# plindhorst/Ray-Tracing-Project

Measured on AMD Instinct MI355X. Metric: Mrays/s (primary) + frame ms at 1920x1080, 1M-tri BVH, 1/2/4/8 GPU, higher is better.
Workload: dtype f32; 1 GPU; C3: 1000000 random triangles (SplitMix64 seed 12345), 1920x1080 primary rays, eye (0,0,1), 1 light; frame=1920x1080, triangles=1000000, mode=primary, parallelism=tiles/1 (one GPU, whole frame), launcher=none, frames_in_flight=4, prewarm_frames=200, hw_queues=4, bvh_nodes=1145398, bvh_depth=26, ref_boxes=4480, builder=sbvh-gpu

## Files before the change

ray-tracing-project_amd/csrc/rt_builders.cpp:

```cpp
#include <atomic>
#include <chrono>
#include <cstdio>
#include <cstdlib>
#include <cstring>
#include <future>

#include "rt_host.h"

namespace rt {
namespace {
struct Prim {
  float lo[3], hi[3], c[3];
  uint32_t id;
};

static bool take_task(std::atomic<int>& live, unsigned cap) {
  if (live.fetch_add(1) < (int)cap) return true;
  live.fetch_sub(1);
  return false;
}

constexpr int kBins = 32;
constexpr float kIsect = 1.0f;
struct Bins {
// ... 88 lines not shown
        const float s = sc[axis];
        const float lo = cb.lo[axis];
        auto it = std::partition(prims.begin() + b, prims.begin() + e, [&](const Prim& p) {
          return std::min(kBins - 1, (int)((p.c[axis] - lo) * s)) <= best_bin;
        });
        mid = (uint32_t)(it - prims.begin());
      }
    } else if ((int)n <= leaf_size) {
      return make_leaf_h();
    }
    if (axis < 0 || mid == b || mid == e) {
      if ((int)n <= kMaxLeaf && !(ext[0] > 0 || ext[1] > 0 || ext[2] > 0)) return make_leaf_h();
      int k = (ext[0] >= ext[1] && ext[0] >= ext[2]) ? 0 : (ext[1] >= ext[2] ? 1 : 2);
      mid = b + n / 2;
      std::nth_element(prims.begin() + b, prims.begin() + mid, prims.begin() + e,
                       [&](const Prim& x, const Prim& y) { return x.c[k] < y.c[k]; });
    }
    const uint32_t me = next.fetch_add(1);
    Aabb lb, rb;
    uint32_t lh, rh;
    if (n > 4096 && depth < 16 && take_task(tasks, hw)) {
      auto fut = std::async(std::launch::async, [&]() { return build(b, mid, depth + 1, lb); });
      rh = build(mid, e, depth + 1, rb);
      lh = fut.get();
      tasks.fetch_sub(1);
    } else {
      lh = build(b, mid, depth + 1, lb);
      rh = build(mid, e, depth + 1, rb);
    }
    Node64 nd{};
    set_child(nd, 0, lb, pad, lh);
    set_child(nd, 1, rb, pad, rh);
    nodes[me] = nd;
    return me;
  }
};

struct SbvhBuilder {
  const HostScene& hs;
  std::vector<Node64>& nodes;
  std::vector<std::vector<uint32_t>> leaf_lists;
  std::atomic<uint32_t> next{0}, nleaf{0};
  std::atomic<int64_t> refs{0};
  int leaf_size = 4;
  float pad = 0.0f, kTrav = 0.7f, alpha = 1e-5f, root_area = 1.0f;
  std::atomic<int> max_depth{0};
  std::atomic<int> tasks{0};
  unsigned hw = 1;

  void verts(uint32_t f, double v[3][3]) const {
    for (int j = 0; j < 3; j++) {
      const f3& w = bound_vert(hs, f, j);
      v[j][0] = w.x; v[j][1] = w.y; v[j][2] = w.z;
    }
  }
  static float down(double x) { float f = (float)x; return (double)f > x ? std::nextafter(f, -INFINITY) : f; }
  static float up(double x) { float f = (float)x; return (double)f < x ? std::nextafter(f, INFINITY) : f; }
  bool clip(uint32_t f, int k, float a, float b, const Prim& within, Prim& out) const {
    double v[3][3];
    verts(f, v);
    double lo[3] = {INFINITY, INFINITY, INFINITY}, hi[3] = {-INFINITY, -INFINITY, -INFINITY};
    auto add = [&](const double* q) {
      for (int i = 0; i < 3; i++) { lo[i] = std::min(lo[i], q[i]); hi[i] = std::max(hi[i], q[i]); }
    };
    for (int j = 0; j < 3; j++) {
      const double* p = v[j];
      const double* q = v[(j + 1) % 3];
      if (p[k] >= a && p[k] <= b) add(p);
      for (double pl : {(double)a, (double)b}) {
        if ((p[k] < pl && q[k] > pl) || (p[k] > pl && q[k] < pl)) {
          const double t = (pl - p[k]) / (q[k] - p[k]);
          double x[3];
          for (int i = 0; i < 3; i++) x[i] = p[i] + t * (q[i] - p[i]);
          x[k] = pl;
          add(x);
        }
      }
    }
    out.id = f;
    for (int i = 0; i < 3; i++) {
      out.lo[i] = std::max(down(lo[i]), within.lo[i]);
      out.hi[i] = std::min(up(hi[i]), within.hi[i]);
      if (i == k) { out.lo[i] = std::max(out.lo[i], a); out.hi[i] = std::min(out.hi[i], b); }
      if (!(out.lo[i] <= out.hi[i])) return false;
      out.c[i] = 0.5f * (out.lo[i] + out.hi[i]);
    }
    return true;
  }

  uint32_t leaf(std::vector<Prim>& r) {
    const uint32_t li = nleaf.fetch_add(1);
    std::vector<uint32_t>& ids = leaf_lists[li];
    ids.reserve(r.size());
    for (const Prim& p : r) ids.push_back(p.id);
    const uint32_t n = (uint32_t)r.size();
    std::vector<Prim>().swap(r);
    return make_leaf(li, n);
  }

  uint32_t build(std::vector<Prim>& r, int depth, Aabb& box, int64_t budget) {
    const uint32_t n = (uint32_t)r.size();
    Aabb cb;
    box = Aabb();
    {
      Aabb pb[16], pc[16];
      const int T = parallel_chunks(n, [&](size_t b, size_t e, int t) {
        Aabb a, c;
        for (size_t i = b; i < e; i++) { a.grow(r[i].lo, r[i].hi); c.growp(r[i].c); }
        pb[t] = a;
        pc[t] = c;
      });
      for (int t = 0; t < T; t++) { box.merge(pb[t]); cb.merge(pc[t]); }
    }
    int md = max_depth.load();
    while (depth > md && !max_depth.compare_exchange_weak(md, depth)) {}
    if (n == 1) return leaf(r);
    const bool forced = depth >= kMaxDepth - 20;
    const float parent_area = std::max(box.area(), 1e-30f);
    const int TB = chunk_count(n);
    std::vector<Bins> part((size_t)TB);
    int o_axis = -1, o_bin = -1;
    float o_cost = INFINITY;
    Aabb o_lb, o_rb;
    float ext[3], sc[3];
    for (int k = 0; k < 3; k++) { ext[k] = cb.hi[k] - cb.lo[k]; sc[k] = ext[k] > 0.0f ? kBins / ext[k] : 0.0f; }
    auto obin = [&](const Prim& p, int k) { return std::min(kBins - 1, (int)((p.c[k] - cb.lo[k]) * sc[k])); };
    if (!forced) {
      for (Bins& B : part) B.clear();
      const int T = parallel_chunks(n, [&](size_t b, size_t e, int t) {
        Bins& B = part[t];
        for (size_t i = b; i < e; i++)
          for (int k = 0; k < 3; k++) {
            if (!(ext[k] > 0.0f)) continue;
            const int bi = obin(r[i], k);
            B.box[k][bi].grow(r[i].lo, r[i].hi);
            B.cnt[k][bi]++;
          }
      });
      for (int t = 1; t < T; t++) part[0].merge(part[t]);
      for (int k = 0; k < 3; k++)
        if (ext[k] > 0.0f) sweep(part[0], k, false, o_cost, o_axis, o_bin, &o_lb, &o_rb);
    }
    int s_axis = -1, s_bin = -1;
    float s_cost = INFINITY;
    float pl[3][kBins + 1];
    float ov = 0.0f;
    if (o_axis >= 0) {
      float d[3];
      for (int k = 0; k < 3; k++) d[k] = std::max(0.0f, std::min(o_lb.hi[k], o_rb.hi[k]) - std::max(o_lb.lo[k], o_rb.lo[k]));
      ov = 2.0f * (d[0] * d[1] + d[1] * d[2] + d[2] * d[0]);
    }
    if (!forced && budget > 0 && (o_axis < 0 || ov > alpha * root_area)) {
      float w[3];
      for (int k = 0; k < 3; k++) {
        w[k] = (box.hi[k] - box.lo[k]) / kBins;
        for (int i = 0; i <= kBins; i++) pl[k][i] = box.lo[k] + w[k] * i;
        pl[k][kBins] = box.hi[k];
      }
      auto sbin = [&](float x, int k) {
        int bi = std::min(kBins - 1, std::max(0, (int)((x - box.lo[k]) / w[k])));
        while (bi > 0 && x < pl[k][bi]) bi--;
        while (bi < kBins - 1 && x >= pl[k][bi + 1]) bi++;
        return bi;
      };
      for (Bins& B : part) B.clear();
      const int T = parallel_chunks(n, [&](size_t b, size_t e, int t) {
        Bins& B = part[t];
        for (size_t i = b; i < e; i++) {
          const Prim& p = r[i];
          for (int k = 0; k < 3; k++) {
            if (!(w[k] > 0.0f)) continue;
            const int b0 = sbin(p.lo[k], k), b1 = sbin(p.hi[k], k);
            B.cnt[k][b0]++;
            B.cnt2[k][b1]++;
            if (b0 == b1) { B.box[k][b0].grow(p.lo, p.hi); continue; }
            for (int bi = b0; bi <= b1; bi++) {
              Prim q;
              if (clip(p.id, k, std::max(pl[k][bi], p.lo[k]), std::min(pl[k][bi + 1], p.hi[k]), p, q)) B.box[k][bi].grow(q.lo, q.hi);
            }
          }
        }
      });
      for (int t = 1; t < T; t++) part[0].merge(part[t]);
      for (int k = 0; k < 3; k++)
        if (w[k] > 0.0f) sweep(part[0], k, true, s_cost, s_axis, s_bin);
    }
    const float best = std::min(o_cost, s_cost);
    if (!forced && (int)n <= leaf_size && (best == INFINITY || (float)n * kIsect <= kTrav + kIsect * best / parent_area))
      return leaf(r);
    if (forced && (int)n <= leaf_size) return leaf(r);
    std::vector<Prim> L, R;
    bool spatial = s_axis >= 0 && s_cost < o_cost;
    const float s_pos = spatial ? pl[s_axis][s_bin + 1] : 0.0f;
    if (spatial) {
      std::vector<int64_t> cnt((size_t)TB, 0);
      const int T = parallel_chunks(n, [&](size_t b, size_t e, int t) {
        int64_t k = 0;
        for (size_t i = b; i < e; i++) k += r[i].lo[s_axis] < s_pos && r[i].hi[s_axis] > s_pos;
        cnt[t] = k;
      });
      int64_t straddle = 0;
      for (int t = 0; t < T; t++) straddle += cnt[t];
      if (straddle > budget) spatial = false;
      else {
        budget -= straddle;
        refs += straddle;
      }
    }
    if (spatial || o_axis >= 0) {
      std::vector<std::vector<Prim>> pL((size_t)TB), pR((size_t)TB);
      const int k = spatial ? s_axis : o_axis;
      const int T = parallel_chunks(n, [&](size_t b, size_t e, int t) {
        std::vector<Prim>& l = pL[t];
        std::vector<Prim>& rr = pR[t];
        for (size_t i = b; i < e; i++) {
          const Prim& p = r[i];
          if (!spatial) { (obin(p, k) <= o_bin ? l : rr).push_back(p); continue; }
          if (p.hi[k] <= s_pos) { l.push_back(p); continue; }
          if (p.lo[k] >= s_pos) { rr.push_back(p); continue; }
          Prim ql, qr;
          const bool hl = clip(p.id, k, p.lo[k], s_pos, p, ql), hr = clip(p.id, k, s_pos, p.hi[k], p, qr);
          if (hl && hr) { l.push_back(ql); rr.push_back(qr); }
          else if (hl) l.push_back(ql);
          else if (hr) rr.push_back(qr);
          else (p.c[k] < s_pos ? l : rr).push_back(p);
        }
      });
      for (int t = 0; t < T; t++) {
        L.insert(L.end(), pL[t].begin(), pL[t].end());
        R.insert(R.end(), pR[t].begin(), pR[t].end());
      }
    }
    if (L.empty() || R.empty()) {
      L.clear();
      R.clear();
      if ((int)n <= kMaxLeaf && !(ext[0] > 0 || ext[1] > 0 || ext[2] > 0)) return leaf(r);
      const int k = (ext[0] >= ext[1] && ext[0] >= ext[2]) ? 0 : (ext[1] >= ext[2] ? 1 : 2);
      std::nth_element(r.begin(), r.begin() + n / 2, r.end(), [&](const Prim& x, const Prim& y) { return x.c[k] < y.c[k]; });
      L.assign(r.begin(), r.begin() + n / 2);
      R.assign(r.begin() + n / 2, r.end());
    }
    std::vector<Prim>().swap(r);
    const uint32_t me = next.fetch_add(1);
    const int64_t bl = (int64_t)((double)budget * (double)L.size() / (double)(L.size() + R.size())), br = budget - bl;
    Aabb lb, rb;
    uint32_t lh, rh;
    if (n > 4096 && depth < 16 && take_task(tasks, hw)) {
      auto fut = std::async(std::launch::async, [&]() { return build(L, depth + 1, lb, bl); });
      rh = build(R, depth + 1, rb, br);
      lh = fut.get();
      tasks.fetch_sub(1);
    } else {
      lh = build(L, depth + 1, lb, bl);
      rh = build(R, depth + 1, rb, br);
    }
    Node64 nd{};
    set_child(nd, 0, lb, pad, lh);
    set_child(nd, 1, rb, pad, rh);
    nodes[me] = nd;
    return me;
  }
};

void build_sbvh(HostScene& hs, int leaf_size, std::vector<Prim>& prims, const Aabb& world, float alpha) {
  const char* budget_env = debug_env("RT_SBVH_BUDGET");
  const float budget = budget_env ? (float)atof(budget_env) : 0.5f;
  const int64_t cap = std::min<int64_t>((int64_t)hs.nf + (int64_t)(budget * hs.nf) + 1, (int64_t)kMaxFaces);
  std::vector<Node64> tmp((size_t)cap);
  SbvhBuilder B{hs, tmp};
  B.hw = std::max(1u, std::thread::hardware_concurrency());
  B.leaf_lists.resize((size_t)cap);
  B.refs = hs.nf;
  B.leaf_size = std::max(1, std::min(leaf_size, kMaxLeaf));
  if (const char* e = debug_env("RT_SAH_TRAV")) B.kTrav = std::max(0.05f, (float)atof(e));
  B.pad = bvh_pad(world.lo, world.hi);
  B.alpha = alpha;
  B.root_area = std::max(world.area(), 1e-30f);
  Aabb rootb;
  const auto tb0 = std::chrono::steady_clock::now();
  uint32_t root = B.build(prims, 0, rootb, cap - hs.nf);
  uint32_t nn = B.next.load();
  if (is_leaf(root)) {
    tmp[0] = wrap_single_leaf_root(rootb, B.pad, root);
    nn = 1;
    root = 0;
  }
  tmp.resize(nn);
  std::vector<uint32_t> order;
  std::vector<uint32_t> st{root};
  while (!st.empty()) {
    Node64& nd = tmp[st.back()];
    st.pop_back();
    uint32_t* hc[2] = {&nd.child0, &nd.child1};
    for (int c = 0; c < 2; c++) {
      const uint32_t h = *hc[c];
      if (!is_leaf(h) || is_sentinel_child(nd, c)) continue;
      const std::vector<uint32_t>& ids = B.leaf_lists[leaf_first(h)];
      *hc[c] = make_leaf((uint32_t)order.size(), leaf_count(h));
      order.insert(order.end(), ids.begin(), ids.end());
    }
    if (!is_leaf(nd.child1)) st.push_back(nd.child1);
    if (!is_leaf(nd.child0)) st.push_back(nd.child0);
  }
  relayout_dfs(hs, tmp, root);
  hs.leaves = (int)B.nleaf.load();
  hs.tris.resize(order.size());
  const float Ro = cert_origin_max(hs);
  parallel_chunks(order.size(), [&](size_t sb, size_t se, int) {
    for (size_t i = sb; i < se; i++) tri_record(hs, order[i], hs.tris[i], Ro);
  });
  if (debug_env("RT_TIMING")) {
    size_t cert = 0;
    for (const TriRec64& t : hs.tris) cert += (t.box & kBoxCertBit) != 0;
    fprintf(stderr, "[rt] sbvh build %.1f ms: %zu references for %d faces, %u nodes, %zu references box-certified\n",
            std::chrono::duration<double, std::milli>(std::chrono::steady_clock::now() - tb0).count(), order.size(),
            hs.nf, nn, cert);
  }
}

}

void build_bvh(HostScene& hs, int leaf_size, bool spatial) {
  hs.nodes.clear();
  hs.tris.clear();
  hs.depth = 0;
  hs.leaves = 0;
  if (hs.nf == 0) { hs.root = 0; return; }
  std::vector<Prim> prims(hs.nf);
  Aabb wparts[16];
  const int TW = parallel_chunks((size_t)hs.nf, [&](size_t b, size_t e, int t) {
    Aabb wa;
    for (size_t f = b; f < e; f++) {
      Prim& p = prims[f];
      p.id = (uint32_t)f;
      for (int k = 0; k < 3; k++) { p.lo[k] = INFINITY; p.hi[k] = -INFINITY; }
      for (int j = 0; j < 3; j++) {
        const f3& w = bound_vert(hs, (uint32_t)f, j);
        const float c[3] = {w.x, w.y, w.z};
        for (int k = 0; k < 3; k++) { p.lo[k] = std::min(p.lo[k], c[k]); p.hi[k] = std::max(p.hi[k], c[k]); }
      }
      for (int k = 0; k < 3; k++) p.c[k] = 0.5f * (p.lo[k] + p.hi[k]);
      wa.grow(p.lo, p.hi);
    }
    wparts[t] = wa;
  });
  Aabb world;
  for (int t = 0; t < TW; t++) world.merge(wparts[t]);
  constexpr float kSbvhAlpha = 1e-3f;
  if (spatial && hs.nf > 1) { build_sbvh(hs, leaf_size, prims, world, kSbvhAlpha); return; }
  std::vector<Node64> tmp((size_t)std::max(hs.nf, 1));
  BvhBuilder B{prims, tmp};
  B.hw = std::max(1u, std::thread::hardware_concurrency());
  B.leaf_size = std::max(1, std::min(leaf_size, kMaxLeaf));
  if (const char* e = debug_env("RT_SAH_TRAV")) B.kTrav = std::max(0.05f, (float)atof(e));
  B.pad = bvh_pad(world.lo, world.hi);
  Aabb rootb;
  const bool timing = debug_env("RT_TIMING") != nullptr;
  auto tb0 = std::chrono::steady_clock::now();
  uint32_t root = B.build(0, (uint32_t)hs.nf, 0, rootb);
  if (timing) fprintf(stderr, "[rt] bvh recursive build %.1f ms\n", std::chrono::duration<double, std::milli>(std::chrono::steady_clock::now() - tb0).count());
  uint32_t nn = B.next.load();
  if (is_leaf(root)) {
    tmp[0] = wrap_single_leaf_root(rootb, B.pad, root);
    nn = 1;
    root = 0;
  }
  tmp.resize(nn);
  relayout_dfs(hs, tmp, root);
  hs.leaves = B.leaves.load();
  hs.tris.resize(hs.nf);
  const float Ro = cert_origin_max(hs);
  parallel_chunks((size_t)hs.nf, [&](size_t sb, size_t se, int) {
    for (size_t s = sb; s < se; s++) tri_record(hs, prims[s].id, hs.tris[s], Ro);
  });
}

}
```

ray-tracing-project_amd/csrc/rt_host.h:

```cpp
#pragma once
#include <algorithm>
#include <cmath>
#include <thread>
#include <vector>

#include "rt_scene.h"

namespace rt {

struct Aabb {
  float lo[3] = {INFINITY, INFINITY, INFINITY}, hi[3] = {-INFINITY, -INFINITY, -INFINITY};
  void grow(const float* l, const float* h) {
    for (int k = 0; k < 3; k++) { lo[k] = std::min(lo[k], l[k]); hi[k] = std::max(hi[k], h[k]); }
  }
  void growp(const float* p) { grow(p, p); }
  void merge(const Aabb& o) { grow(o.lo, o.hi); }
  float area() const {
    float d[3];
    for (int k = 0; k < 3; k++) d[k] = std::max(0.0f, hi[k] - lo[k]);
    return 2.0f * (d[0] * d[1] + d[1] * d[2] + d[2] * d[0]);
  }
};

inline int chunk_count(size_t n) {
  return n >= 65536 ? (int)std::max(1u, std::min(16u, std::thread::hardware_concurrency())) : 1;
}
template <typename F>
int parallel_chunks(size_t b, size_t e, F&& f) {
  const size_t n = e - b;
  const int T = chunk_count(n);
  std::vector<std::thread> th;
  for (int t = 1; t < T; t++) th.emplace_back([&, t]() { f(b + n * t / T, b + n * (t + 1) / T, t); });
  f(b, b + n / T, 0);
  for (auto& x : th) x.join();
  return T;
}
template <typename F>
int parallel_chunks(size_t n, F&& f) { return parallel_chunks(0, n, f); }

inline void set_child(Node64& n, int c, const float lo[3], const float hi[3], float pad, uint32_t h) {
  if (c == 0) {
    n.c0lx = lo[0] - pad; n.c0hx = hi[0] + pad; n.c0ly = lo[1] - pad; n.c0hy = hi[1] + pad; n.c0lz = lo[2] - pad; n.c0hz = hi[2] + pad;
    n.child0 = h;
  } else {
    n.c1lx = lo[0] - pad; n.c1hx = hi[0] + pad; n.c1ly = lo[1] - pad; n.c1hy = hi[1] + pad; n.c1lz = lo[2] - pad; n.c1hz = hi[2] + pad;
    n.child1 = h;
  }
}
inline void set_child(Node64& n, int c, const Aabb& b, float pad, uint32_t h) { set_child(n, c, b.lo, b.hi, pad, h); }

struct ChildBox {
  float lo[3], hi[3];
  uint32_t h;
};
inline ChildBox child_box(const Node64& n, int c) {
  if (c == 0) return {{n.c0lx, n.c0ly, n.c0lz}, {n.c0hx, n.c0hy, n.c0hz}, n.child0};
  return {{n.c1lx, n.c1ly, n.c1lz}, {n.c1hx, n.c1hy, n.c1hz}, n.child1};
}

inline bool is_sentinel_child(const Node64& n, int c) { return (c ? n.c1lx : n.c0lx) > (c ? n.c1hx : n.c0hx); }
inline Node64 wrap_single_leaf_root(const Aabb& box, float pad, uint32_t leaf) {
  Node64 nd{};
  set_child(nd, 0, box, pad, leaf);
  nd.c1lx = nd.c1ly = nd.c1lz = INFINITY;
  nd.c1hx = nd.c1hy = nd.c1hz = -INFINITY;
  nd.child1 = make_leaf(0, 1);
  return nd;
}

void build_ref_boxes(HostScene& hs, const float* v4, int32_t min_faces, int32_t max_boxes);
void assign_box_ranks(HostScene& hs);
void build_bvh(HostScene& hs, int leaf_size, bool spatial);
float bvh_pad(const float lo[3], const float hi[3]);
bool model_is_similarity(const float* M);
void tri_record(const HostScene& hs, uint32_t f, TriRec64& r, float Ro);
void relayout_dfs(HostScene& hs, const std::vector<Node64>& tmp, uint32_t root);
bool build_bvh_gpu(HostScene& hs, int device, int leaf_size, double* gpu_ms);
bool build_bvh_ploc(HostScene& hs, int device, int leaf_size, double* gpu_ms);
bool build_bvh_sah_gpu(HostScene& hs, int device, int leaf_size, bool spatial, double* gpu_ms);
void build_bvh4(HostScene& hs);

}
```

ray-tracing-project_amd/csrc/rt_layout.cpp:

```cpp
#include <atomic>
#include <cstdio>
#include <cstdlib>
#include <cstring>
#include <functional>

#include "rt_host.h"

namespace rt {

static bool safe_normal(const HostScene& hs, uint32_t f) {
  const f3& w0 = hs.wv[hs.fidx[3 * f]];
  const f3& w1 = hs.wv[hs.fidx[3 * f + 1]];
  const f3& w2 = hs.wv[hs.fidx[3 * f + 2]];
  const f3 e0 = sub(w1, w0), e2 = sub(w0, w2);
  const float A = norm(cross(e0, neg(e2))) / 2;
  if (!(A > 1e-30f) || !std::isfinite(A)) return false;
  const f3& n = hs.fnn[f];
  for (int k = 0; k < 3; k++) {
    const f3& nk = hs.vnn[hs.fidx[3 * f + k]];
    if (!std::isfinite(nk.x) || !std::isfinite(nk.y) || !std::isfinite(nk.z)) return false;
    if (std::fabs(sqnorm(nk) - 1.0f) > 1e-3f) return false;
    if (!(dot(n, nk) >= 0.5f)) return false;
  }
  return true;
// ... 50 lines not shown
  for (float v : hs.ov3) R = std::max(R, std::fabs(v));
  return std::isfinite(R) ? 16.0f * R : 0.0f;
}

constexpr double kCertNormalSin = 1e-3;
bool model_is_similarity(const float* M) {
  double c[3][3], n2[3];
  for (int j = 0; j < 3; j++) {
    for (int k = 0; k < 3; k++) c[j][k] = M[4 * j + k];
    n2[j] = c[j][0] * c[j][0] + c[j][1] * c[j][1] + c[j][2] * c[j][2];
    if (!std::isfinite(n2[j]) || !(n2[j] > 0.0)) return false;
  }
  for (int j = 0; j < 3; j++) {
    if (std::fabs(n2[j] - n2[0]) > 1e-5 * n2[0]) return false;
    const int i = (j + 1) % 3;
    const double d = c[j][0] * c[i][0] + c[j][1] * c[i][1] + c[j][2] * c[i][2];
    if (std::fabs(d) > 1e-5 * n2[0]) return false;
  }
  return M[3] == 0.0f && M[7] == 0.0f && M[11] == 0.0f && M[15] == 1.0f;
}

static double face_normal_tilt(const HostScene& hs, uint32_t f) {
  double w[3][3];
  for (int j = 0; j < 3; j++) {
    const f3& p = hs.wv[hs.fidx[3 * f + j]];
    w[j][0] = p.x; w[j][1] = p.y; w[j][2] = p.z;
  }
  const double a[3] = {w[1][0] - w[0][0], w[1][1] - w[0][1], w[1][2] - w[0][2]};
  const double c[3] = {w[2][0] - w[0][0], w[2][1] - w[0][1], w[2][2] - w[0][2]};
  const double g[3] = {a[1] * c[2] - a[2] * c[1], a[2] * c[0] - a[0] * c[2], a[0] * c[1] - a[1] * c[0]};
  const f3& nf = hs.fnn[f];
  const double n[3] = {nf.x, nf.y, nf.z};
  const double gg = g[0] * g[0] + g[1] * g[1] + g[2] * g[2], nn = n[0] * n[0] + n[1] * n[1] + n[2] * n[2];
  if (!std::isfinite(gg) || !std::isfinite(nn) || !(gg > 0.0) || !(nn > 0.0)) return 2.0;
  const double x[3] = {g[1] * n[2] - g[2] * n[1], g[2] * n[0] - g[0] * n[2], g[0] * n[1] - g[1] * n[0]};
  const double dn = g[0] * n[0] + g[1] * n[1] + g[2] * n[2];
  if (!(dn > 0.0)) return 2.0;
  return std::sqrt((x[0] * x[0] + x[1] * x[1] + x[2] * x[2]) / (gg * nn));
}

constexpr double kBoundTilt = 1e-6;
void accept_region(HostScene& hs) {
  hs.av.clear();
  std::atomic<bool> any{false};
  parallel_chunks((size_t)hs.nf, [&](size_t b, size_t e, int) {
    for (size_t f = b; f < e && !any.load(std::memory_order_relaxed); f++)
      if (!(face_normal_tilt(hs, (uint32_t)f) <= kBoundTilt)) any = true;
  });
  if (!any) return;
  hs.av.resize(3 * (size_t)hs.nf);
  parallel_chunks((size_t)hs.nf, [&](size_t b, size_t e, int) {
    for (size_t f = b; f < e; f++) {
      const f3& nf = hs.fnn[f];
      const double n[3] = {nf.x, nf.y, nf.z}, nn = n[0] * n[0] + n[1] * n[1] + n[2] * n[2];
      const bool tilted = !(face_normal_tilt(hs, (uint32_t)f) <= kBoundTilt);
      for (int j = 0; j < 3; j++) {
        const f3& w = hs.wv[hs.fidx[3 * f + j]];
        f3& p = hs.av[3 * f + j];
        p = w;
        if (!tilted || !(nn > 0.0) || !std::isfinite(nn)) continue;
        const double s = (n[0] * w.x + n[1] * w.y + n[2] * w.z - (double)hs.fdist[f]) / nn;
        p = f3{(float)(w.x - s * n[0]), (float)(w.y - s * n[1]), (float)(w.z - s * n[2])};
      }
    }
  });
}

static bool box_certified(const HostScene& hs, uint32_t f, float Ro) {
  if (!(Ro > 0.0f) || hs.ov3.empty()) return false;
  const double tilt = face_normal_tilt(hs, f);
  if (!(tilt <= kCertNormalSin)) return false;
  const RefBox& b = hs.boxes[hs.face_box[f]];
  double v[3][3];
  for (int j = 0; j < 3; j++)
    for (int k = 0; k < 3; k++) {
      v[j][k] = hs.ov3[3 * (size_t)hs.fidx[3 * f + j] + k];
      if (!std::isfinite(v[j][k])) return false;
    }
  double L[3];
  for (int j = 0; j < 3; j++) {
    const double* a = v[j];
    const double* c = v[(j + 1) % 3];
    L[j] = std::sqrt((c[0] - a[0]) * (c[0] - a[0]) + (c[1] - a[1]) * (c[1] - a[1]) + (c[2] - a[2]) * (c[2] - a[2]));
  }
  const double diam = std::max(L[0], std::max(L[1], L[2]));
  if (!(diam > 0.0)) return false;
  for (int j = 0; j < 3; j++) {
    const double a = L[(j + 1) % 3], c = L[(j + 2) % 3], o = L[j];
    if (!(a > 0.0 && c > 0.0)) return false;
    const double cosv = std::min(1.0, std::max(-1.0, (a * a + c * c - o * o) / (2.0 * a * c)));
    const double s_half = std::sqrt(std::max(0.0, (1.0 - cosv) / 2.0));
    if (!(s_half >= 0.01)) return false;
  }
  for (int k = 0; k < 3; k++) {
    const double lo = b.low[k], hi = b.high[k];
    if (!std::isfinite(lo) || !std::isfinite(hi)) return false;
    const double S = (hi - lo) + std::fabs(lo) + std::fabs(hi);
    const double need = 1e-5 * (S + Ro) + 1e-30 + 1e-5 * S + 4e-4 * diam + 2.0 * tilt * diam;
    for (int j = 0; j < 3; j++)
      if (!(v[j][k] - lo >= need && hi - v[j][k] >= need)) return false;
  }
  return true;
}

uint32_t tri_flags(const HostScene& hs, uint32_t f, float Ro) {
  return (safe_normal(hs, f) ? kSafeNormalBit : 0u) | (box_certified(hs, f, Ro) ? kBoxCertBit : 0u);
}

void tri_record(const HostScene& hs, uint32_t f, TriRec64& r, float Ro) {
  const f3& n = hs.fnn[f];
  const f3& w0 = hs.wv[hs.fidx[3 * f]];
  const f3& w1 = hs.wv[hs.fidx[3 * f + 1]];
  const f3& w2 = hs.wv[hs.fidx[3 * f + 2]];
  r.nx = n.x; r.ny = n.y; r.nz = n.z; r.dist = hs.fdist[f];
  r.w0x = w0.x; r.w0y = w0.y; r.w0z = w0.z;
  r.w1x = w1.x; r.w1y = w1.y; r.w1z = w1.z;
  r.w2x = w2.x; r.w2y = w2.y; r.w2z = w2.z;
  r.rank = hs.face_rank[f];
  r.face = f;
  r.box = hs.face_box[f] | tri_flags(hs, f, Ro);
}

static void face_records(const HostScene& hs, std::vector<TriRec64>& out) {
  out.resize(hs.nf);
  const float Ro = cert_origin_max(hs);
  parallel_chunks((size_t)hs.nf, [&](size_t b, size_t e, int) {
    for (size_t f = b; f < e; f++) tri_record(hs, (uint32_t)f, out[f], Ro);
  });
}

static void set_verts(TriRec64& r, const f3& w0, const f3& w1, const f3& w2) {
  r.w0x = w0.x; r.w0y = w0.y; r.w0z = w0.z;
  r.w1x = w1.x; r.w1y = w1.y; r.w1z = w1.z;
  r.w2x = w2.x; r.w2y = w2.y; r.w2z = w2.z;
}
static void bound_records(const HostScene& hs, std::vector<TriRec64>& recs) {
  if (hs.av.empty()) return;
  parallel_chunks(recs.size(), [&](size_t b, size_t e, int) {
    for (size_t i = b; i < e; i++) {
      TriRec64& r = recs[i];
      set_verts(r, bound_vert(hs, r.face, 0), bound_vert(hs, r.face, 1), bound_vert(hs, r.face, 2));
    }
  });
}
static bool device_buildable(const std::vector<TriRec64>& recs) {
  std::atomic<bool> ok{true};
  parallel_chunks(recs.size(), [&](size_t b, size_t e, int) {
    for (size_t i = b; i < e && ok.load(std::memory_order_relaxed); i++) {
      const TriRec64& r = recs[i];
      const float v[9] = {r.w0x, r.w0y, r.w0z, r.w1x, r.w1y, r.w1z, r.w2x, r.w2y, r.w2z};
      for (float x : v)
        if (!(std::fabs(x) <= 1e30f)) ok = false;
    }
  });
  return ok.load();
}
static void world_records(HostScene& hs) {
  if (hs.av.empty()) return;
  parallel_chunks(hs.tris.size(), [&](size_t b, size_t e, int) {
    for (size_t i = b; i < e; i++) {
      TriRec64& r = hs.tris[i];
      const uint32_t* v = &hs.fidx[3 * (size_t)r.face];
      set_verts(r, hs.wv[v[0]], hs.wv[v[1]], hs.wv[v[2]]);
    }
  });
}

static uint32_t octant_order(const Node64& nd) {
  const float c0[3] = {nd.c0lx + nd.c0hx, nd.c0ly + nd.c0hy, nd.c0lz + nd.c0hz};
  const float c1[3] = {nd.c1lx + nd.c1hx, nd.c1ly + nd.c1hy, nd.c1lz + nd.c1hz};
  int axis = 0;
  float best = -1.0f;
  for (int k = 0; k < 3; k++) {
    const float sep = std::fabs(c1[k] - c0[k]);
    if (sep > best) best = sep, axis = k;
  }
  const bool c1_low = c1[axis] < c0[axis];
  uint32_t bits = 0;
  for (uint32_t oct = 0; oct < 8; oct++) {
    const bool negative = (oct >> axis) & 1u;
    if (c1_low != negative) bits |= 1u << oct;
  }
  return bits;
}

static void relayout_pairs(HostScene& hs, const std::vector<Node64>& tmp, uint32_t root) {
  Node64 empty;
  memset(&empty, 0, sizeof empty);
  empty.c0lx = empty.c0ly = empty.c0lz = empty.c1lx = empty.c1ly = empty.c1lz = INFINITY;
  empty.c0hx = empty.c0hy = empty.c0hz = empty.c1hx = empty.c1hy = empty.c1hz = -INFINITY;
  empty.child0 = empty.child1 = make_leaf(0, 1);
  std::vector<uint32_t> remap(tmp.size(), UINT32_MAX);
  std::vector<uint32_t> slot_src{root, UINT32_MAX};
  remap[root] = 0;
  std::vector<std::pair<uint32_t, int>> st{{root, 1}};
  int depth = 0;
  while (!st.empty()) {
    const auto [n, d] = st.back();
    st.pop_back();
    depth = std::max(depth, d + 1);
    const Node64& nd = tmp[n];
    const bool i0 = !is_leaf(nd.child0), i1 = !is_leaf(nd.child1);
    if (!i0 && !i1) continue;
    const uint32_t base = (uint32_t)slot_src.size();
    slot_src.push_back(UINT32_MAX);
    slot_src.push_back(UINT32_MAX);
    uint32_t k = base;
    if (i0) { remap[nd.child0] = k; slot_src[k++] = nd.child0; }
    if (i1) { remap[nd.child1] = k; slot_src[k++] = nd.child1; }
    if (i1) st.push_back({nd.child1, d + 1});
    if (i0) st.push_back({nd.child0, d + 1});
  }
  hs.nodes.resize(slot_src.size());
  hs.leaves = 0;
  for (size_t i = 0; i < slot_src.size(); i++) {
    if (slot_src[i] == UINT32_MAX) { hs.nodes[i] = empty; continue; }
    Node64 nd = tmp[slot_src[i]];
    if (!is_leaf(nd.child0)) nd.child0 = remap[nd.child0];
    if (!is_leaf(nd.child1)) nd.child1 = remap[nd.child1];
    hs.leaves += (int)is_leaf(nd.child0) + (int)is_leaf(nd.child1);
    nd.pad0 = octant_order(nd);
    hs.nodes[i] = nd;
  }
  hs.root = 0;
  hs.depth = depth;
}

void relayout_dfs(HostScene& hs, const std::vector<Node64>& tmp, uint32_t root) {
  const char* layout_env = debug_env("RT_NODE_LAYOUT");
  const bool pairs = layout_env && !strcmp(layout_env, "pairs");
  if (pairs) { relayout_pairs(hs, tmp, root); return; }
  const size_t N = tmp.size();
  std::vector<uint32_t> remap(N, UINT32_MAX), order;
  int depth = 0;
  bool forward = root < N;
  std::vector<uint32_t> size(N, 1);
  for (size_t i = N; forward && i-- > 0;) {
    const Node64& nd = tmp[i];
    for (uint32_t c : {nd.child0, nd.child1}) {
      if (is_leaf(c)) continue;
      if (c <= i || c >= N) { forward = false; break; }
      size[i] += size[c];
    }
  }
  if (forward) {
    std::vector<uint8_t> lev(N, 0);
    remap[root] = 0;
    lev[root] = 1;
    order.assign(size[root], UINT32_MAX);
    for (size_t i = root; i < N; i++) {
      const uint32_t p = remap[i];
      if (p == UINT32_MAX) continue;
      order[p] = (uint32_t)i;
      depth = std::max(depth, lev[i] + 1);
      const Node64& nd = tmp[i];
      uint32_t next = p + 1;
      for (uint32_t c : {nd.child0, nd.child1}) {
        if (is_leaf(c)) continue;
        remap[c] = next;
        lev[c] = (uint8_t)std::min(lev[i] + 1, 255);
        next += size[c];
      }
    }
  } else {
    std::fill(remap.begin(), remap.end(), UINT32_MAX);
    std::vector<std::pair<uint32_t, int>> st{{root, 1}};
    while (!st.empty()) {
      const auto [n, d] = st.back();
      st.pop_back();
      remap[n] = (uint32_t)order.size();
      order.push_back(n);
      depth = std::max(depth, d + 1);
      const Node64& nd = tmp[n];
      if (!is_leaf(nd.child1)) st.push_back({nd.child1, d + 1});
      if (!is_leaf(nd.child0)) st.push_back({nd.child0, d + 1});
    }
  }
  hs.nodes.resize(order.size());
  int leaves[16] = {};
  const int T = parallel_chunks(order.size(), [&](size_t b, size_t e, int t) {
    int lv = 0;
    for (size_t i = b; i < e; i++) {
      Node64 nd = tmp[order[i]];
      if (!is_leaf(nd.child0)) nd.child0 = remap[nd.child0];
      if (!is_leaf(nd.child1)) nd.child1 = remap[nd.child1];
      lv += (int)is_leaf(nd.child0) + (int)is_leaf(nd.child1);
      nd.pad0 = octant_order(nd);
      hs.nodes[i] = nd;
    }
    leaves[t] = lv;
  });
  hs.root = 0;
  hs.depth = depth;
  hs.leaves = 0;
  for (int t = 0; t < T; t++) hs.leaves += leaves[t];
}

static bool gpu_build_inputs(const HostScene& hs, float lo[3], float hi[3], std::vector<TriRec64>& recs) {
  world_bounds(hs, lo, hi);
  face_records(hs, recs);
  bound_records(hs, recs);
  return device_buildable(recs);
}
static bool adopt_tree(HostScene& hs, const std::vector<Node64>& tmp, std::vector<TriRec64>& tris,
                       const std::function<void(int)>& accepted = nullptr, PhaseTimer* pt = nullptr) {
  HostScene trial;
  relayout_dfs(trial, tmp, 0);
  if (trial.depth > kMaxDepth + 2) return false;
  if (accepted) accepted(trial.depth);
  hs.nodes = std::move(trial.nodes);
  hs.root = 0;
  hs.depth = trial.depth;
  hs.leaves = trial.leaves;
  hs.tris = std::move(tris);
  if (pt) pt->mark("tris");
  world_records(hs);
  if (pt) pt->mark("world_records");
  return true;
}

bool build_bvh_gpu(HostScene& hs, int device, int leaf_size, double* gpu_ms) {
  if (hs.nf <= leaf_size || hs.nf < 2) return false;
  float lo[3], hi[3];
  std::vector<TriRec64> recs, tris;
  if (!gpu_build_inputs(hs, lo, hi, recs)) return false;
  std::vector<Node64> tmp;
  if (gpu_build_lbvh(device, recs, lo, hi, std::max(1, std::min(leaf_size, kMaxLeaf)), bvh_pad(lo, hi), tmp, tris,
                     gpu_ms) != RT_OK)
    return false;
  return adopt_tree(hs, tmp, tris);
}

constexpr int kPlocRadius = 4;
constexpr float kPlocTrav = 0.7f;
bool build_bvh_ploc(HostScene& hs, int device, int leaf_size, double* gpu_ms) {
  if (hs.nf < 2) return false;
  float lo[3], hi[3];
  std::vector<TriRec64> recs;
  if (!gpu_build_inputs(hs, lo, hi, recs)) return false;
  std::vector<int32_t> child;
  std::vector<float> box;
  std::vector<uint8_t> leaf;
  int iters = 0;
  const int lb = std::max(1, std::min(leaf_size, kMaxLeaf));
  int radius = kPlocRadius, rule = 0;
  float trav = kPlocTrav;
  if (const char* e = debug_env("RT_PLOC_RADIUS")) radius = std::max(1, std::min(32, atoi(e)));
  if (const char* e = debug_env("RT_PLOC_TRAV")) trav = std::max(0.05f, (float)atof(e));
  if (const char* e = debug_env("RT_PLOC_RULE")) rule = atoi(e);
  if (gpu_build_ploc(device, recs, lo, hi, lb, radius, trav, child, box, leaf, gpu_ms, &iters, rule) != RT_OK)
    return false;
  const int n = hs.nf, ni = n - 1, root = n - 2;
  const float pad = bvh_pad(lo, hi);
  std::vector<uint32_t> handle_int((size_t)ni, 0), handle_tri((size_t)n, 0);
  std::vector<int32_t> kept;
  std::vector<TriRec64> tris;
  tris.reserve((size_t)n);
  std::vector<int32_t> st{root}, sub;
  auto tri_of = [&](int32_t c) { return (uint32_t)~c; };
  while (!st.empty()) {
    const int32_t c = st.back();
    st.pop_back();
    if (c < 0) {
      handle_tri[tri_of(c)] = make_leaf((uint32_t)tris.size(), 1u);
      tris.push_back(recs[tri_of(c)]);
    } else if (leaf[(size_t)c] && c != root) {
      const uint32_t first = (uint32_t)tris.size();
      sub.assign(1, c);
      while (!sub.empty()) {
        const int32_t q = sub.back();
        sub.pop_back();
        if (q < 0) { tris.push_back(recs[tri_of(q)]); continue; }
        sub.push_back(child[2 * (size_t)q + 1]);
        sub.push_back(child[2 * (size_t)q]);
      }
      handle_int[(size_t)c] = make_leaf(first, (uint32_t)tris.size() - first);
    } else {
      handle_int[(size_t)c] = (uint32_t)kept.size();
      kept.push_back(c);
      st.push_back(child[2 * (size_t)c + 1]);
      st.push_back(child[2 * (size_t)c]);
    }
  }
  std::vector<Node64> tmp(kept.size());
  for (size_t k = 0; k < kept.size(); k++) {
    const int32_t q = kept[k];
    Node64 nd{};
    for (int side = 0; side < 2; side++) {
      const int32_t c = child[2 * (size_t)q + side];
      float b[6];
      uint32_t h;
      if (c < 0) {
        const TriRec64& t = recs[tri_of(c)];
        b[0] = std::min(std::min(t.w0x, t.w1x), t.w2x); b[3] = std::max(std::max(t.w0x, t.w1x), t.w2x);
        b[1] = std::min(std::min(t.w0y, t.w1y), t.w2y); b[4] = std::max(std::max(t.w0y, t.w1y), t.w2y);
        b[2] = std::min(std::min(t.w0z, t.w1z), t.w2z); b[5] = std::max(std::max(t.w0z, t.w1z), t.w2z);
        h = handle_tri[tri_of(c)];
      } else {
        for (int j = 0; j < 6; j++) b[j] = box[6 * (size_t)c + j];
        h = handle_int[(size_t)c];
      }
      set_child(nd, side, b, b + 3, pad, h);
    }
    tmp[k] = nd;
  }
  return adopt_tree(hs, tmp, tris, [&](int depth) {
    if (debug_env("RT_TIMING")) fprintf(stderr, "[rt] ploc: %d iterations, %zu nodes, depth %d\n", iters, tmp.size(), depth);
  });
}

bool build_bvh_sah_gpu(HostScene& hs, int device, int leaf_size, bool spatial, double* gpu_ms) {
  if (hs.nf < 2) return false;
  PhaseTimer pt("sbvh-gpu");
  float lo[3], hi[3];
  std::vector<TriRec64> recs;
  if (!gpu_build_inputs(hs, lo, hi, recs)) return false;
  pt.mark("records");
  std::vector<uint32_t> nchild, slot_face;
  std::vector<float> ncb;
  int levels = 0;
  float trav = 0.7f;
  if (const char* e = debug_env("RT_SAH_TRAV")) trav = std::max(0.05f, (float)atof(e));
  float budget = 0.5f;
  if (const char* e = debug_env("RT_SBVH_BUDGET")) budget = std::max(0.0f, (float)atof(e));
  constexpr float kSbvhGpuAlpha = 1e-3f;
  if (gpu_build_sah(device, recs, lo, hi, std::max(1, std::min(leaf_size, kMaxLeaf)), trav, spatial, budget, kSbvhGpuAlpha,
                    nchild, ncb, slot_face, gpu_ms, &levels) != RT_OK)
    return false;
  pt.mark("gpu_build_sah");
  const size_t nn = nchild.size() / 2;
  const float pad = bvh_pad(lo, hi);
  std::vector<Node64> tmp(nn);
  std::atomic<bool> bad{false};
  parallel_chunks(nn, [&](size_t kb, size_t ke, int) {
    for (size_t k = kb; k < ke; k++) {
      Node64 nd{};
      for (int side = 0; side < 2; side++) {
        const float* b = &ncb[12 * k + 6 * side];
        const uint32_t h = nchild[2 * k + side];
        if (!is_leaf(h) && h >= nn) bad = true;
        set_child(nd, side, b, b + 3, pad, h);
      }
      tmp[k] = nd;
    }
  });
  if (bad) return false;
  pt.mark("nodes");
  std::vector<TriRec64> tris;
  return adopt_tree(hs, tmp, tris, [&](int depth) {
    pt.mark("relayout");
    if (debug_env("RT_TIMING"))
      fprintf(stderr, "[rt] %s: %d levels, %zu nodes, %zu references, depth %d\n", spatial ? "sbvh-gpu" : "sah-gpu", levels, nn,
              slot_face.size(), depth);
    tris.resize(slot_face.size());
    parallel_chunks(slot_face.size(), [&](size_t b, size_t e, int) {
      for (size_t sl = b; sl < e; sl++) tris[sl] = recs[slot_face[sl]];
    });
  }, &pt);
}

namespace {
float warea(const ChildBox& w) {
  float d[3];
  for (int k = 0; k < 3; k++) d[k] = std::max(0.0f, w.hi[k] - w.lo[k]);
  return d[0] * d[1] + d[1] * d[2] + d[2] * d[0];
}

void quantize(Node4Q& q, const ChildBox* ch, int n) {
  float L[3] = {INFINITY, INFINITY, INFINITY}, U[3] = {-INFINITY, -INFINITY, -INFINITY};
  for (int c = 0; c < n; c++)
    for (int k = 0; k < 3; k++) { L[k] = std::min(L[k], ch[c].lo[k]); U[k] = std::max(U[k], ch[c].hi[k]); }
  uint8_t eb[3];
  double scale[3];
  for (int k = 0; k < 3; k++) {
    const double ext = (double)U[k] - (double)L[k];
    int e = -100;
    if (ext > 0) {
      e = (int)std::ceil(std::log2(ext / 255.0));
      while (std::ldexp(255.0, e) < ext) e++;
      e = std::max(e, -100);
    }
    eb[k] = (uint8_t)(e + 127);
    scale[k] = std::ldexp(1.0, e);
  }
  q.ox = L[0]; q.oy = L[1]; q.oz = L[2];
  q.ex = eb[0]; q.ey = eb[1]; q.ez = eb[2];
  q.valid = 0;
  uint32_t* ql[3] = {&q.qlx, &q.qly, &q.qlz};
  uint32_t* qh[3] = {&q.qhx, &q.qhy, &q.qhz};
  for (int k = 0; k < 3; k++) { *ql[k] = 0; *qh[k] = 0; }
  const double org[3] = {q.ox, q.oy, q.oz};
  for (int c = 0; c < 4; c++) {
    if (c >= n) { q.child[c] = 0; continue; }
    q.valid |= (uint8_t)(1u << c);
    q.child[c] = ch[c].h;
    for (int k = 0; k < 3; k++) {
      double a = std::floor(((double)ch[c].lo[k] - org[k]) / scale[k]);
      double b = std::ceil(((double)ch[c].hi[k] - org[k]) / scale[k]);
      a = std::min(std::max(a, 0.0), 255.0);
      b = std::min(std::max(b, 0.0), 255.0);
      while (a > 0 && org[k] + a * scale[k] > (double)ch[c].lo[k]) a -= 1;
      while (b < 255 && org[k] + b * scale[k] < (double)ch[c].hi[k]) b += 1;
      *ql[k] |= (uint32_t)a << (8 * c);
      *qh[k] |= (uint32_t)b << (8 * c);
    }
  }
  q.pad0 = q.pad1 = 0;
}

template <typename Rec, typename Emit>
uint32_t collapse(const std::vector<Node64>& bin, uint32_t n2, std::vector<Rec>& out, int depth, int& maxd, Emit&& emit) {
  maxd = std::max(maxd, depth);
  ChildBox ch[4] = {child_box(bin[n2], 0), child_box(bin[n2], 1)};
  int n = is_sentinel_child(bin[n2], 1) ? 1 : 2;
  while (n < 4) {
    int best = -1;
    float ba = -1.0f;
    for (int c = 0; c < n; c++)
      if (!is_leaf(ch[c].h) && warea(ch[c]) > ba) { ba = warea(ch[c]); best = c; }
    if (best < 0) break;
    const Node64& sub = bin[ch[best].h];
    ch[best] = child_box(sub, 0);
    ch[n++] = child_box(sub, 1);
  }
  const uint32_t me = (uint32_t)out.size();
  out.emplace_back();
  for (int c = 0; c < n; c++)
    if (!is_leaf(ch[c].h)) ch[c].h = collapse(bin, ch[c].h, out, depth + 1, maxd, emit);
  emit(out[me], ch, n);
  return me;
}
}

void build_bvh4(HostScene& hs) {
  hs.nodes4.clear();
  hs.depth4 = 0;
  if (hs.nodes.empty()) return;
  hs.nodes4.reserve(hs.nodes.size() / 2 + 1);
  int maxd = 0;
  collapse(hs.nodes, hs.root, hs.nodes4, 0, maxd, quantize);
  hs.depth4 = maxd + 1;
}

namespace {
bool wide_before(const float* a, const float* b, uint32_t oct) {
  int axis = 0;
  float best = -1.0f;
  for (int k = 0; k < 3; k++) {
    const float sep = std::fabs((b[2 * k] + b[2 * k + 1]) - (a[2 * k] + a[2 * k + 1]));
    if (sep > best) best = sep, axis = k;
  }
  const float ca = a[2 * axis] + a[2 * axis + 1], cb = b[2 * axis] + b[2 * axis + 1];
  return ((oct >> axis) & 1u) ? ca > cb : ca < cb;
}

void wide_record(Wide4& w, const ChildBox* ch, int n) {
  memset(&w, 0, sizeof w);
  w.n = (uint8_t)n;
  for (int c = 0; c < 4; c++) {
    for (int k = 0; k < 3; k++) {
      w.box[c][2 * k] = c < n ? ch[c].lo[k] : INFINITY;
      w.box[c][2 * k + 1] = c < n ? ch[c].hi[k] : -INFINITY;
    }
    w.child[c] = c < n ? ch[c].h : kWideEmpty;
  }
  for (uint32_t oct = 0; oct < 8; oct++) {
    uint8_t* o = w.order[oct];
    for (int c = 0; c < 4; c++) o[c] = (uint8_t)c;
    for (int i = 1; i < n; i++)
      for (int j = i; j > 0 && wide_before(w.box[o[j]], w.box[o[j - 1]], oct); j--) std::swap(o[j], o[j - 1]);
  }
}
}

void build_wide(HostScene& hs) {
  hs.wide.clear();
  hs.depth_wide = 0;
  if (hs.nodes.empty() || is_leaf(hs.root)) return;
  hs.wide.reserve(hs.nodes.size() / 2 + 1);
  int maxd = 0;
  collapse(hs.nodes, hs.root, hs.wide, 0, maxd, wide_record);
  hs.depth_wide = maxd + 1;
  if (3 * hs.depth_wide + 4 > kStackW) {
    hs.wide.clear();
    hs.depth_wide = 0;
  }
}

}
```

Baseline: 10490 Mrays/s.

## Add SAH-driven tree rotation optimizer after SBVH builds

```diff
diff --git a/ray-tracing-project_amd/csrc/rt_builders.cpp b/ray-tracing-project_amd/csrc/rt_builders.cpp
--- a/ray-tracing-project_amd/csrc/rt_builders.cpp
+++ b/ray-tracing-project_amd/csrc/rt_builders.cpp
@@ -414,6 +414,12 @@
     if (!is_leaf(nd.child1)) st.push_back(nd.child1);
     if (!is_leaf(nd.child0)) st.push_back(nd.child0);
   }
+  std::vector<uint32_t> slot_order;
+  if (optimize_tree(tmp, root, tree_opt_rounds(true), tree_opt_slots() ? &slot_order : nullptr) && !slot_order.empty()) {
+    std::vector<uint32_t> by_slot(order.size());
+    for (size_t i = 0; i < order.size(); i++) by_slot[i] = order[slot_order[i]];
+    order.swap(by_slot);
+  }
   relayout_dfs(hs, tmp, root);
   hs.leaves = (int)B.nleaf.load();
   hs.tris.resize(order.size());
@@ -478,12 +484,14 @@
     root = 0;
   }
   tmp.resize(nn);
+  std::vector<uint32_t> slot_order;
+  optimize_tree(tmp, root, tree_opt_rounds(false), tree_opt_slots() ? &slot_order : nullptr);
   relayout_dfs(hs, tmp, root);
   hs.leaves = B.leaves.load();
   hs.tris.resize(hs.nf);
   const float Ro = cert_origin_max(hs);
   parallel_chunks((size_t)hs.nf, [&](size_t sb, size_t se, int) {
-    for (size_t s = sb; s < se; s++) tri_record(hs, prims[s].id, hs.tris[s], Ro);
+    for (size_t s = sb; s < se; s++) tri_record(hs, prims[slot_order.empty() ? s : slot_order[s]].id, hs.tris[s], Ro);
   });
 }
 
diff --git a/ray-tracing-project_amd/csrc/rt_host.h b/ray-tracing-project_amd/csrc/rt_host.h
--- a/ray-tracing-project_amd/csrc/rt_host.h
+++ b/ray-tracing-project_amd/csrc/rt_host.h
@@ -71,6 +71,12 @@
 void build_ref_boxes(HostScene& hs, const float* v4, int32_t min_faces, int32_t max_boxes);
 void assign_box_ranks(HostScene& hs);
 void build_bvh(HostScene& hs, int leaf_size, bool spatial);
+constexpr int kTreeOptRounds = 2;
+constexpr int kTreeOptRetries = 3;
+constexpr int kTreeOptSlots = 1;
+int tree_opt_rounds(bool on_by_default);
+bool tree_opt_slots();
+bool optimize_tree(std::vector<Node64>& nodes, uint32_t& root, int rounds, std::vector<uint32_t>* slot_order);
 float bvh_pad(const float lo[3], const float hi[3]);
 bool model_is_similarity(const float* M);
 void tri_record(const HostScene& hs, uint32_t f, TriRec64& r, float Ro);
diff --git a/ray-tracing-project_amd/csrc/rt_layout.cpp b/ray-tracing-project_amd/csrc/rt_layout.cpp
--- a/ray-tracing-project_amd/csrc/rt_layout.cpp
+++ b/ray-tracing-project_amd/csrc/rt_layout.cpp
@@ -376,17 +376,28 @@
   bound_records(hs, recs);
   return device_buildable(recs);
 }
-static bool adopt_tree(HostScene& hs, const std::vector<Node64>& tmp, std::vector<TriRec64>& tris,
-                       const std::function<void(int)>& accepted = nullptr, PhaseTimer* pt = nullptr) {
+static bool adopt_tree(HostScene& hs, std::vector<Node64>& tmp, std::vector<TriRec64>& tris,
+                       const std::function<void(int)>& accepted = nullptr, PhaseTimer* pt = nullptr, bool optimise = false) {
+  uint32_t root = 0;
+  std::vector<uint32_t> slot_order;
+  optimize_tree(tmp, root, tree_opt_rounds(optimise), tree_opt_slots() ? &slot_order : nullptr);
+  if (pt) pt->mark("tree_opt");
   HostScene trial;
-  relayout_dfs(trial, tmp, 0);
+  relayout_dfs(trial, tmp, root);
   if (trial.depth > kMaxDepth + 2) return false;
   if (accepted) accepted(trial.depth);
   hs.nodes = std::move(trial.nodes);
   hs.root = 0;
   hs.depth = trial.depth;
   hs.leaves = trial.leaves;
-  hs.tris = std::move(tris);
+  if (slot_order.empty()) {
+    hs.tris = std::move(tris);
+  } else {
+    hs.tris.resize(slot_order.size());
+    parallel_chunks(slot_order.size(), [&](size_t b, size_t e, int) {
+      for (size_t sl = b; sl < e; sl++) hs.tris[sl] = tris[slot_order[sl]];
+    });
+  }
   if (pt) pt->mark("tris");
   world_records(hs);
   if (pt) pt->mark("world_records");
@@ -530,7 +541,7 @@
     parallel_chunks(slot_face.size(), [&](size_t b, size_t e, int) {
       for (size_t sl = b; sl < e; sl++) tris[sl] = recs[slot_face[sl]];
     });
-  }, &pt);
+  }, &pt, spatial);
 }
 
 namespace {
diff --git a/ray-tracing-project_amd/csrc/rt_optimize.cpp b/ray-tracing-project_amd/csrc/rt_optimize.cpp
--- /dev/null
+++ b/ray-tracing-project_amd/csrc/rt_optimize.cpp
@@ -0,0 +1,323 @@
+#include <atomic>
+#include <chrono>
+#include <cstdio>
+#include <cstdlib>
+
+#include "rt_host.h"
+
+namespace rt {
+namespace {
+constexpr uint32_t kNone = UINT32_MAX;
+
+struct Ent {
+  float lo[3], hi[3];
+  uint32_t c[2];
+};
+struct Move {
+  float gain = 0.0f;
+  uint32_t x = kNone, pivot = kNone;
+};
+
+inline float area_of(const float* lo, const float* hi) {
+  float d[3];
+  for (int k = 0; k < 3; k++) d[k] = std::max(0.0f, hi[k] - lo[k]);
+  return 2.0f * (d[0] * d[1] + d[1] * d[2] + d[2] * d[0]);
+}
+inline float area(const Ent& e) { return area_of(e.lo, e.hi); }
+inline float union_area(const Ent& a, const Ent& b) {
+  float lo[3], hi[3];
+  for (int k = 0; k < 3; k++) { lo[k] = std::min(a.lo[k], b.lo[k]); hi[k] = std::max(a.hi[k], b.hi[k]); }
+  return area_of(lo, hi);
+}
+inline bool finite_box(const Ent& e) {
+  for (int k = 0; k < 3; k++)
+    if (!std::isfinite(e.lo[k]) || !std::isfinite(e.hi[k])) return false;
+  return true;
+}
+
+struct Tree {
+  uint32_t N = 0;
+  std::vector<Ent> ent;
+  std::vector<uint32_t> parent;
+  std::vector<uint32_t> handle;
+  std::vector<uint32_t> order;
+  std::vector<uint8_t> level, height;
+  int depth = 0;
+  double inner = 0.0;
+
+  uint32_t size() const { return (uint32_t)ent.size(); }
+  bool leaf(uint32_t e) const { return e >= N; }
+  uint32_t sibling(uint32_t p, uint32_t c) const { return ent[p].c[0] == c ? ent[p].c[1] : ent[p].c[0]; }
+
+  bool refresh() {
+    const uint32_t E = size();
+    order.clear();
+    order.reserve(E);
+    level.assign(E, 0);
+    height.assign(E, 0);
+    std::vector<uint32_t> st{0};
+    level[0] = 1;
+    while (!st.empty()) {
+      const uint32_t e = st.back();
+      st.pop_back();
+      if (order.size() >= E) return false;
+      order.push_back(e);
+      if (leaf(e)) continue;
+      for (int k = 1; k >= 0; k--) {
+        const uint32_t c = ent[e].c[k];
+        if (c >= E || level[c] != 0 || parent[c] != e) return false;
+        level[c] = (uint8_t)std::min(level[e] + 1, 255);
+        st.push_back(c);
+      }
+    }
+    if (order.size() != E) return false;
+    depth = 0;
+    inner = 0.0;
+    for (size_t i = E; i-- > 0;) {
+      const uint32_t e = order[i];
+      if (leaf(e)) { depth = std::max(depth, (int)level[e]); continue; }
+      Ent& n = ent[e];
+      const Ent &a = ent[n.c[0]], &b = ent[n.c[1]];
+      for (int k = 0; k < 3; k++) { n.lo[k] = std::min(a.lo[k], b.lo[k]); n.hi[k] = std::max(a.hi[k], b.hi[k]); }
+      height[e] = (uint8_t)std::min(std::max(height[n.c[0]], height[n.c[1]]) + 1, 255);
+      inner += area(n);
+    }
+    return true;
+  }
+
+  Move search(uint32_t n, int max_level, std::vector<std::pair<uint32_t, float>>& st) const {
+    Move best;
+    const uint32_t p = parent[n];
+    const Ent& bn = ent[n];
+    if (!finite_box(bn)) return best;
+    const float An = area(bn);
+    const int hn = height[n];
+    float D = area(ent[p]);
+    Ent pb;
+    for (int k = 0; k < 3; k++) { pb.lo[k] = INFINITY; pb.hi[k] = -INFINITY; }
+    uint32_t out = n;
+    for (uint32_t piv = p; piv != kNone; out = piv, piv = parent[piv]) {
+      const uint32_t sib = sibling(piv, out);
+      const int lift = piv == p ? 1 : 0;
+      st.clear();
+      st.push_back({sib, 0.0f});
+      while (!st.empty()) {
+        const auto [x, induced] = st.back();
+        st.pop_back();
+        if (!(D - induced - An > best.gain)) continue;
+        const Ent& bx = ent[x];
+        const float direct = union_area(bx, bn);
+        if (!(lift && x == sib)) {
+          const float gain = D - induced - direct;
+          if (gain > best.gain && std::isfinite(gain) && finite_box(bx) &&
+              (int)level[x] - lift + 1 + std::max(hn, (int)height[x]) <= max_level) {
+            best.gain = gain;
+            best.x = x;
+            best.pivot = piv;
+          }
+        }
+        if (leaf(x)) continue;
+        const float below = induced + (direct - area(bx));
+        if (!(D - below - An > best.gain)) continue;
+        const uint32_t c0 = bx.c[0], c1 = bx.c[1];
+        const float g0 = union_area(ent[c0], bn) - area(ent[c0]), g1 = union_area(ent[c1], bn) - area(ent[c1]);
+        if (g0 <= g1) { st.push_back({c1, below}); st.push_back({c0, below}); }
+        else { st.push_back({c0, below}); st.push_back({c1, below}); }
+      }
+      const Ent& bs = ent[sib];
+      for (int k = 0; k < 3; k++) { pb.lo[k] = std::min(pb.lo[k], bs.lo[k]); pb.hi[k] = std::max(pb.hi[k], bs.hi[k]); }
+      if (piv != p) D += area(ent[piv]) - area(pb);
+    }
+    return best;
+  }
+
+  void replace_child(uint32_t p, uint32_t from, uint32_t to) {
+    ent[p].c[ent[p].c[0] == from ? 0 : 1] = to;
+    parent[to] = p;
+  }
+  void apply(uint32_t n, uint32_t x) {
+    const uint32_t p = parent[n], s = sibling(p, n), g = parent[p];
+    replace_child(g, p, s);
+    replace_child(parent[x], x, p);
+    ent[p].c[ent[p].c[0] == n ? 1 : 0] = x;
+    parent[x] = p;
+  }
+};
+}
+
+int tree_opt_rounds(bool on_by_default) { return knob_int("RT_TREE_OPT", on_by_default ? kTreeOptRounds : 0, 0, 64); }
+bool tree_opt_slots() { return knob_int("RT_TREE_OPT_SLOTS", kTreeOptSlots, 0, 1) != 0; }
+
+bool optimize_tree(std::vector<Node64>& nodes, uint32_t& root, int rounds, std::vector<uint32_t>* slot_order) {
+  if (slot_order) slot_order->clear();
+  if (rounds <= 0 || nodes.empty() || root >= nodes.size()) return false;
+  const auto t0 = std::chrono::steady_clock::now();
+  PhaseTimer pt("tree_opt");
+  Tree T;
+  std::vector<uint32_t> src;
+  {
+    size_t nl = 0;
+    std::vector<uint32_t> st{root};
+    std::vector<uint8_t> seen(nodes.size(), 0);
+    while (!st.empty()) {
+      const uint32_t i = st.back();
+      st.pop_back();
+      if (i >= nodes.size() || seen[i]) return false;
+      seen[i] = 1;
+      src.push_back(i);
+      const Node64& nd = nodes[i];
+      if (is_sentinel_child(nd, 0) || is_sentinel_child(nd, 1)) return false;
+      nl += (size_t)is_leaf(nd.child0) + (size_t)is_leaf(nd.child1);
+      if (!is_leaf(nd.child1)) st.push_back(nd.child1);
+      if (!is_leaf(nd.child0)) st.push_back(nd.child0);
+    }
+    if (nl < 4) return false;
+    T.N = (uint32_t)src.size();
+    std::vector<uint32_t> id(nodes.size(), kNone);
+    for (uint32_t e = 0; e < T.N; e++) id[src[e]] = e;
+    T.ent.resize(T.N + nl);
+    T.parent.assign(T.N + nl, kNone);
+    T.handle.reserve(nl);
+    for (uint32_t e = 0; e < T.N; e++) {
+      const Node64& nd = nodes[src[e]];
+      for (int c = 0; c < 2; c++) {
+        const ChildBox cb = child_box(nd, c);
+        const uint32_t ce = is_leaf(cb.h) ? T.N + (uint32_t)T.handle.size() : id[cb.h];
+        if (is_leaf(cb.h)) T.handle.push_back(cb.h);
+        Ent& x = T.ent[ce];
+        for (int k = 0; k < 3; k++) { x.lo[k] = cb.lo[k]; x.hi[k] = cb.hi[k]; }
+        if (is_leaf(cb.h)) x.c[0] = x.c[1] = kNone;
+        T.ent[e].c[c] = ce;
+        T.parent[ce] = e;
+      }
+    }
+  }
+  if (!T.refresh()) return false;
+  pt.mark("setup");
+  const int depth0 = T.depth;
+  const double inner0 = T.inner;
+  const uint32_t E = T.size();
+  const int max_level = kMaxDepth;
+  std::vector<Move> best(E);
+  std::vector<uint32_t> claimed(E, 0), cand(E), movers, losers, frozen_parent, path;
+  std::vector<std::pair<uint32_t, uint32_t>> undo;
+  int64_t moves = 0;
+  int done = 0, searches = 0;
+  uint32_t stamp = 0;
+  bool stop = false;
+  const int retries = knob_int("RT_TREE_OPT_RETRIES", kTreeOptRetries, 0, 64);
+  for (int r = 1; r <= rounds && !stop; r++) {
+    cand.resize(E);
+    for (uint32_t n = 0; n < E; n++) cand[n] = n;
+    for (int sub = 0; sub <= retries && !cand.empty(); sub++) {
+      const uint32_t C = (uint32_t)cand.size();
+      std::atomic<uint32_t> next{0};
+      constexpr uint32_t kBlock = 1024;
+      parallel_chunks(C, [&](size_t, size_t, int) {
+        std::vector<std::pair<uint32_t, float>> st;
+        st.reserve(256);
+        for (;;) {
+          const uint32_t b = next.fetch_add(kBlock);
+          if (b >= C) break;
+          for (uint32_t i = b; i < std::min(C, b + kBlock); i++) {
+            const uint32_t n = cand[i], p = T.parent[n];
+            best[n] = p == kNone || T.parent[p] == kNone ? Move() : T.search(n, max_level, st);
+          }
+        }
+      });
+      searches++;
+      pt.mark("search");
+      movers.clear();
+      for (const uint32_t n : cand)
+        if (best[n].x != kNone && best[n].gain > 0.0f) movers.push_back(n);
+      if (movers.empty()) { cand.clear(); break; }
+      std::sort(movers.begin(), movers.end(), [&](uint32_t a, uint32_t b) {
+        return best[a].gain != best[b].gain ? best[a].gain > best[b].gain : a < b;
+      });
+      frozen_parent = T.parent;
+      const double inner_before = T.inner;
+      stamp++;
+      undo.clear();
+      losers.clear();
+      for (const uint32_t n : movers) {
+        const Move& m = best[n];
+        path.clear();
+        path.push_back(n);
+        bool free_path = true;
+        for (const uint32_t from : {frozen_parent[n], m.x})
+          for (uint32_t a = from; free_path; a = frozen_parent[a]) {
+            if (a == kNone) { free_path = false; break; }
+            path.push_back(a);
+            if (a == m.pivot) break;
+          }
+        path.push_back(frozen_parent[frozen_parent[n]]);
+        for (size_t i = 0; free_path && i < path.size(); i++) free_path = claimed[path[i]] != stamp;
+        if (!free_path) { losers.push_back(n); continue; }
+        for (const uint32_t a : path) claimed[a] = stamp;
+        undo.push_back({n, T.sibling(T.parent[n], n)});
+        T.apply(n, m.x);
+      }
+      pt.mark("resolve");
+      const bool sound = T.refresh();
+      pt.mark("refresh");
+      if (!sound || T.depth > std::max(depth0, max_level) || !(T.inner <= inner_before)) {
+        for (size_t i = undo.size(); i-- > 0;) T.apply(undo[i].first, undo[i].second);
+        if (!T.refresh()) return false;
+        stop = true;
+        break;
+      }
+      moves += (int64_t)undo.size();
+      done = r;
+      if (debug_env("RT_TIMING"))
+        fprintf(stderr, "[rt] tree_opt round %d.%d: %u searched, %zu gain, %zu moved, summed area %.6g -> %.6g, depth %d\n", r,
+                sub, C, movers.size(), undo.size(), inner_before, T.inner, T.depth);
+      std::sort(losers.begin(), losers.end());
+      cand.swap(losers);
+    }
+  }
+  if (moves == 0) return false;
+  std::vector<Node64> outn(T.N);
+  std::vector<uint32_t> pos(E, kNone);
+  {
+    uint32_t k = 0;
+    for (const uint32_t e : T.order)
+      if (!T.leaf(e)) pos[e] = k++;
+  }
+  if (slot_order) {
+    uint32_t first = 0;
+    for (const uint32_t e : T.order) {
+      if (!T.leaf(e)) continue;
+      uint32_t& h = T.handle[e - T.N];
+      const uint32_t cnt = leaf_count(h);
+      for (uint32_t i = 0; i < cnt; i++) slot_order->push_back(leaf_first(h) + i);
+      h = make_leaf(first, cnt);
+      first += cnt;
+    }
+  }
+  parallel_chunks(E, [&](size_t b, size_t e, int) {
+    for (size_t i = b; i < e; i++) {
+      if (pos[i] == kNone) continue;
+      Node64 nd{};
+      for (int c = 0; c < 2; c++) {
+        const uint32_t ce = T.ent[i].c[c];
+        const Ent& x = T.ent[ce];
+        set_child(nd, c, x.lo, x.hi, 0.0f, T.leaf(ce) ? T.handle[ce - T.N] : pos[ce]);
+      }
+      outn[pos[i]] = nd;
+    }
+  });
+  nodes.swap(outn);
+  root = 0;
+  if (debug_env("RT_TIMING")) {
+    double k_trav = 0.7, leafc = 0.0;
+    if (const char* e = debug_env("RT_SAH_TRAV")) k_trav = std::max(0.05, atof(e));
+    for (uint32_t e = T.N; e < E; e++) leafc += (double)area(T.ent[e]) * leaf_count(T.handle[e - T.N]);
+    const double ra = area(T.ent[0]);
+    fprintf(stderr, "[rt] tree_opt %.1f ms: %d rounds (%d searches), %lld moves of %u entities, SAH %.2f -> %.2f, depth %d -> %d\n",
+            std::chrono::duration<double, std::milli>(std::chrono::steady_clock::now() - t0).count(), done, searches, (long long)moves,
+            E, ra > 0 ? (k_trav * inner0 + leafc) / ra : 0.0, ra > 0 ? (k_trav * T.inner + leafc) / ra : 0.0, depth0, T.depth);
+  }
+  return true;
+}
+
+}
```

New measurement: 10460 Mrays/s. About the same (-0.3%).
